# open-rmf/rmf_crowdsim

Hardware: NVIDIA B200
Metric: agent-steps/sec (query+Zanlungo+integrate) (higher is better)
Workload: dtype f64

## Files before the change

### bindings/rust/rmf_crowdsim_gpu-sys/src/lib.rs

```rust
#![allow(non_camel_case_types)]
use std::os::raw::{c_char, c_int};

#[repr(C)]
pub struct rcs_sim {
    _private: [u8; 0],
}

pub const RCS_OK: c_int = 0;
pub const RCS_ERR_OUT_OF_BOUNDS: c_int = 1;
pub const RCS_ERR_SPAWN: c_int = 2;
pub const RCS_ERR_CUDA: c_int = 3;
pub const RCS_ERR_NCCL: c_int = 4;
pub const RCS_ERR_CAPACITY: c_int = 5;
pub const RCS_ERR_ARG: c_int = 6;
pub const RCS_ERR_NO_DEVICE: c_int = 7;
pub const RCS_ERR_HALO: c_int = 8;
pub const RCS_ORDER_STORAGE: u32 = 0;
pub const RCS_ORDER_ID: u32 = 1;
pub const RCS_STEP_DEFAULT: u32 = 0;
pub const RCS_STEP_NO_COMMIT: u32 = 1;

#[repr(C)]
pub struct rcs_sim_desc {
    pub width: f64,
    pub height: f64,
    pub cell_size: f64,
    pub offset_x: f64,
    pub offset_y: f64,
    pub capacity: u64,
    pub device: i32,
    pub flags: u32,
}

#[repr(C)]
#[derive(Default, Debug, Clone, Copy)]
pub struct rcs_stats {
    pub n_agents: u64,
    pub oob_count: u64,
    pub first_oob_id: u64,
    pub nonfinite_count: u64,
    pub finite_tti_count: u64,
    pub neighbour_total: u64,
    pub candidate_total: u64,
    pub spawned: u64,
    pub destroyed: u64,
    pub steps: u64,
}

#[repr(C)]
pub struct rcs_source_sink_desc {
    pub source_x: f64,
    pub source_y: f64,
    pub radius_sink: f64,
    pub monotonic_rate: f64,
    pub hl: u32,
    pub lp: u32,
    pub n_waypoints: u64,
    pub waypoints_xy: *const f64,
    pub loop_forever: i32,
    pub agent_eyesight_range: f64,
}

extern "C" {
    pub fn rcs_abi_version() -> u32;
    pub fn rcs_sim_create(desc: *const rcs_sim_desc, out: *mut *mut rcs_sim) -> c_int;
    pub fn rcs_sim_destroy(sim: *mut rcs_sim);
    pub fn rcs_last_error(sim: *const rcs_sim) -> *const c_char;

    pub fn rcs_lp_none(sim: *mut rcs_sim, out_lp: *mut u32) -> c_int;
    pub fn rcs_lp_zanlungo(sim: *mut rcs_sim, agent_scale: f64, obstacle_scale: f64, reaction_time: f64,
                           force_distance: f64, agent_mass: f64, agent_radius: f64, out_lp: *mut u32) -> c_int;
    pub fn rcs_hl_constant(sim: *mut rcs_sim, vx: f64, vy: f64, out_hl: *mut u32) -> c_int;
    pub fn rcs_hl_parity(sim: *mut rcs_sim, vx: f64, vy: f64, out_hl: *mut u32) -> c_int;
    pub fn rcs_hl_host(sim: *mut rcs_sim, out_hl: *mut u32) -> c_int;
    pub fn rcs_hl_none(sim: *mut rcs_sim, out_hl: *mut u32) -> c_int;
    pub fn rcs_hl_route(sim: *mut rcs_sim, n_points: u64, xy: *const f64, out_hl: *mut u32) -> c_int;
    pub fn rcs_hl_route_set_target(sim: *mut rcs_sim, n: u64, ids: *const u64) -> c_int;
    pub fn rcs_hl_route_table(sim: *mut rcs_sim, n_legs: u64, targets_xy: *const f64, leg_points: *const u64,
                              xy: *const f64, out_hl: *mut u32) -> c_int;
    pub fn rcs_hl_route_table_set_target(sim: *mut rcs_sim, hl: u32, n: u64, ids: *const u64,
                                         targets_xy: *const f64) -> c_int;

    pub fn rcs_add_agents(sim: *mut rcs_sim, n: u64, xy: *const f64, hl: u32, lp: u32, eyesight: f64,
                          out_ids: *mut u64) -> c_int;
    pub fn rcs_remove_agents(sim: *mut rcs_sim, n: u64, ids: *const u64) -> c_int;
    pub fn rcs_set_state(sim: *mut rcs_sim, n: u64, ids: *const u64, x: *const f64, y: *const f64,
                         vx: *const f64, vy: *const f64) -> c_int;
    pub fn rcs_set_preferred_velocity(sim: *mut rcs_sim, n: u64, ids: *const u64, vxy: *const f64) -> c_int;
    pub fn rcs_read_agents(sim: *mut rcs_sim, order: u32, cap: u64, ids: *mut u64, x: *mut f64, y: *mut f64,
                           vx: *mut f64, vy: *mut f64, next_waypoint: *mut u32, out_n: *mut u64) -> c_int;
    pub fn rcs_read_agents_async(sim: *mut rcs_sim, order: u32, cap: u64, ids: *mut u64, x: *mut f64,
                                 y: *mut f64, vx: *mut f64, vy: *mut f64, out_n: *mut u64) -> c_int;
    pub fn rcs_read_wait(sim: *mut rcs_sim) -> c_int;
    pub fn rcs_agent_count(sim: *mut rcs_sim, out_n: *mut u64) -> c_int;

    pub fn rcs_step(sim: *mut rcs_sim, secs: u64, nanos: u32) -> c_int;
    pub fn rcs_step_async(sim: *mut rcs_sim, secs: u64, nanos: u32, flags: u32) -> c_int;
    pub fn rcs_sync(sim: *mut rcs_sim) -> c_int;
    pub fn rcs_step_stats(sim: *mut rcs_sim, out: *mut rcs_stats) -> c_int;
    pub fn rcs_step_in_loop(sim: *mut rcs_sim, secs: u64, nanos: u32, order: *const u64, n_order: u64,
                            max_sweeps: u32, out_sweeps: *mut u32) -> c_int;
    pub fn rcs_poll_events(sim: *mut rcs_sim, spawned_cap: u64, spawned_ids: *mut u64, spawned_xy: *mut f64,
                           n_spawned: *mut u64, destroyed_cap: u64, destroyed_ids: *mut u64,
                           n_destroyed: *mut u64) -> c_int;
    pub fn rcs_add_source_sink(sim: *mut rcs_sim, desc: *const rcs_source_sink_desc, out_id: *mut u64) -> c_int;
    pub fn rcs_remove_source_sink(sim: *mut rcs_sim, id: u64) -> c_int;

    pub fn rcs_cell_of(sim: *mut rcs_sim, n: u64, xy: *const f64, out_idx: *mut i64) -> c_int;
    pub fn rcs_index_add_or_update(sim: *mut rcs_sim, n: u64, ids: *const u64, xy: *const f64) -> c_int;
    pub fn rcs_index_remove(sim: *mut rcs_sim, n: u64, ids: *const u64) -> c_int;
    pub fn rcs_query_radius(sim: *mut rcs_sim, nq: u64, qxy: *const f64, radius: *const f64, offsets: *mut u64,
                            out_ids: *mut u64, ids_cap: u64) -> c_int;
    pub fn rcs_query_knn(sim: *mut rcs_sim, nq: u64, qxy: *const f64, k: u64, out_ids: *mut u64,
                         out_counts: *mut u64) -> c_int;

    pub fn rcs_set_option(sim: *mut rcs_sim, option: u32, value: u64) -> c_int;
    pub fn rcs_graph_stats(sim: *mut rcs_sim, out_graph_launches: *mut u64, out_captures: *mut u64) -> c_int;

    pub fn rcs_nccl_unique_id(out_id: *mut u8) -> c_int;
    pub fn rcs_dist_init(sim: *mut rcs_sim, rank: i32, world: i32, nccl_id: *const u8, halo_capacity: u64) -> c_int;
    pub fn rcs_dist_set_boundaries(sim: *mut rcs_sim, world: i32, bounds: *const u64) -> c_int;
    pub fn rcs_dist_reserve_ids(sim: *mut rcs_sim, next_id: u64) -> c_int;
    pub fn rcs_dist_peer_export(sim: *mut rcs_sim, out_handle: *mut u8) -> c_int;
    pub fn rcs_dist_peer_connect(sim: *mut rcs_sim, left_handle: *const u8, right_handle: *const u8) -> c_int;
    pub fn rcs_dist_peer_disable(sim: *mut rcs_sim) -> c_int;
    pub fn rcs_dist_strip(sim: *mut rcs_sim, rank: i32, world: i32, c0: *mut u64, c1: *mut u64) -> c_int;
    pub fn rcs_dist_add_agents(sim: *mut rcs_sim, n: u64, ids: *const u64, xy: *const f64, vxy: *const f64,
                               hl: u32, lp: u32, eyesight: f64) -> c_int;
}
```

### include/rcs.h

```cpp
#ifndef RCS_H_
#define RCS_H_

#include <stdint.h>

#ifdef __cplusplus
extern "C" {
#endif

#define RCS_ABI_VERSION 1

typedef struct rcs_sim rcs_sim;

enum {
  RCS_OK = 0,
  RCS_ERR_OUT_OF_BOUNDS = 1,
  RCS_ERR_SPAWN = 2,
  RCS_ERR_CUDA = 3,
  RCS_ERR_NCCL = 4,
  RCS_ERR_CAPACITY = 5,
  RCS_ERR_ARG = 6,
  RCS_ERR_NO_DEVICE = 7,
  RCS_ERR_HALO = 8
};

typedef struct rcs_sim_desc {
  double width;
  double height;
  double cell_size;
  double offset_x;
  double offset_y;
  uint64_t capacity;
  int32_t device;
  uint32_t flags;
} rcs_sim_desc;

typedef struct rcs_stats {
  uint64_t n_agents;
  uint64_t oob_count;
  uint64_t first_oob_id;
  uint64_t nonfinite_count;
  uint64_t finite_tti_count;
  uint64_t neighbour_total;
  uint64_t candidate_total;
  uint64_t spawned;
  uint64_t destroyed;
  uint64_t steps;
} rcs_stats;

uint32_t rcs_abi_version(void);

int rcs_sim_create(const rcs_sim_desc* desc, rcs_sim** out);
void rcs_sim_destroy(rcs_sim* sim);
const char* rcs_last_error(const rcs_sim* sim);


int rcs_lp_none(rcs_sim* sim, uint32_t* out_lp);
int rcs_lp_zanlungo(rcs_sim* sim, double agent_scale, double obstacle_scale, double reaction_time,
                    double force_distance, double agent_mass, double agent_radius, uint32_t* out_lp);

int rcs_hl_constant(rcs_sim* sim, double vx, double vy, uint32_t* out_hl);
int rcs_hl_parity(rcs_sim* sim, double vx, double vy, uint32_t* out_hl);
int rcs_hl_host(rcs_sim* sim, uint32_t* out_hl);
int rcs_hl_route(rcs_sim* sim, uint64_t n_points, const double* xy, uint32_t* out_hl);
int rcs_hl_route_set_target(rcs_sim* sim, uint64_t n, const uint64_t* ids);
int rcs_hl_route_table(rcs_sim* sim, uint64_t n_legs, const double* targets_xy, const uint64_t* leg_points,
                       const double* xy, uint32_t* out_hl);
int rcs_hl_route_table_set_target(rcs_sim* sim, uint32_t hl, uint64_t n, const uint64_t* ids,
                                  const double* targets_xy);
int rcs_hl_none(rcs_sim* sim, uint32_t* out_hl);


int rcs_add_agents(rcs_sim* sim, uint64_t n, const double* xy, uint32_t hl, uint32_t lp, double eyesight,
                   uint64_t* out_ids);
int rcs_remove_agents(rcs_sim* sim, uint64_t n, const uint64_t* ids);
int rcs_set_state(rcs_sim* sim, uint64_t n, const uint64_t* ids, const double* x, const double* y,
                  const double* vx, const double* vy);
int rcs_set_preferred_velocity(rcs_sim* sim, uint64_t n, const uint64_t* ids, const double* vxy);

#define RCS_ORDER_STORAGE 0u
#define RCS_ORDER_ID 1u
int rcs_read_agents(rcs_sim* sim, uint32_t order, uint64_t cap, uint64_t* ids, double* x, double* y, double* vx,
                    double* vy, uint32_t* next_waypoint, uint64_t* out_n);
int rcs_agent_count(rcs_sim* sim, uint64_t* out_n);
int rcs_read_agents_async(rcs_sim* sim, uint32_t order, uint64_t cap, uint64_t* ids, double* x, double* y, double* vx,
                          double* vy, uint64_t* out_n);
int rcs_read_wait(rcs_sim* sim);


#define RCS_STEP_DEFAULT 0u
#define RCS_STEP_NO_COMMIT 1u

int rcs_step(rcs_sim* sim, uint64_t secs, uint32_t nanos);
int rcs_step_async(rcs_sim* sim, uint64_t secs, uint32_t nanos, uint32_t flags);
int rcs_sync(rcs_sim* sim);
int rcs_step_stats(rcs_sim* sim, rcs_stats* out);

int rcs_step_in_loop(rcs_sim* sim, uint64_t secs, uint32_t nanos, const uint64_t* order, uint64_t n_order,
                     uint32_t max_sweeps, uint32_t* out_sweeps);

int rcs_poll_events(rcs_sim* sim, uint64_t spawned_cap, uint64_t* spawned_ids, double* spawned_xy,
                    uint64_t* n_spawned, uint64_t destroyed_cap, uint64_t* destroyed_ids, uint64_t* n_destroyed);

typedef struct rcs_source_sink_desc {
  double source_x, source_y;
  double radius_sink;
  double monotonic_rate;
  uint32_t hl, lp;
  uint64_t n_waypoints;
  const double* waypoints_xy;
  int32_t loop_forever;
  double agent_eyesight_range;
} rcs_source_sink_desc;
int rcs_add_source_sink(rcs_sim* sim, const rcs_source_sink_desc* desc, uint64_t* out_id);
int rcs_remove_source_sink(rcs_sim* sim, uint64_t id);


int rcs_cell_of(rcs_sim* sim, uint64_t n, const double* xy, int64_t* out_idx);
int rcs_index_add_or_update(rcs_sim* sim, uint64_t n, const uint64_t* ids, const double* xy);
int rcs_index_remove(rcs_sim* sim, uint64_t n, const uint64_t* ids);
int rcs_query_radius(rcs_sim* sim, uint64_t nq, const double* qxy, const double* radius, uint64_t* offsets,
                     uint64_t* out_ids, uint64_t ids_cap);
int rcs_query_knn(rcs_sim* sim, uint64_t nq, const double* qxy, uint64_t k, uint64_t* out_ids,
                  uint64_t* out_counts);

int rcs_set_trace(rcs_sim* sim, int32_t on);
int rcs_trace_sizes(rcs_sim* sim, uint64_t* n_agents, uint64_t* n_neighbours);
int rcs_read_trace(rcs_sim* sim, uint64_t* ids, double* t_i, double* fx, double* fy, uint64_t* nb_offsets,
                   uint64_t* nb_ids);

#define RCS_OPT_STEP_KERNEL 1u
#define RCS_OPT_GRAPHS 3u
int rcs_set_option(rcs_sim* sim, uint32_t option, uint64_t value);

#define RCS_NUM_EVENTS 64u
int rcs_event_record(rcs_sim* sim, uint32_t slot);
int rcs_event_elapsed_ms(rcs_sim* sim, uint32_t start_slot, uint32_t stop_slot, float* out_ms);
int rcs_host_alloc(uint64_t bytes, void** out);
int rcs_host_free(void* p);
int rcs_flush_l2(rcs_sim* sim, uint64_t bytes);
int rcs_kernel_timing(rcs_sim* sim, int32_t on);
int rcs_kernel_time_ms(rcs_sim* sim, double* out_ms, uint64_t* out_launches);
int rcs_launch_count(rcs_sim* sim, uint64_t* out);
int rcs_graph_stats(rcs_sim* sim, uint64_t* out_graph_launches, uint64_t* out_captures);
int rcs_fp64_peak(int32_t device, double* out_tflops, double* out_dadd_tops);

int rcs_nccl_unique_id(uint8_t out_id[128]);
int rcs_dist_init(rcs_sim* sim, int32_t rank, int32_t world, const uint8_t nccl_id[128], uint64_t halo_capacity);
int rcs_dist_set_boundaries(rcs_sim* sim, int32_t world, const uint64_t* bounds);
int rcs_dist_peer_export(rcs_sim* sim, uint8_t out_handle[64]);
int rcs_dist_peer_connect(rcs_sim* sim, const uint8_t* left_handle, const uint8_t* right_handle);
int rcs_dist_peer_disable(rcs_sim* sim);
int rcs_dist_strip(rcs_sim* sim, int32_t rank, int32_t world, uint64_t* c0, uint64_t* c1);
int rcs_dist_add_agents(rcs_sim* sim, uint64_t n, const uint64_t* ids, const double* xy, const double* vxy,
                        uint32_t hl, uint32_t lp, double eyesight);
int rcs_dist_reserve_ids(rcs_sim* sim, uint64_t next_id);
int rcs_dist_init_local(rcs_sim** sims, int32_t world, uint64_t halo_capacity);
int rcs_dist_step_local(rcs_sim** sims, int32_t world, uint64_t secs, uint32_t nanos, uint32_t flags);

#ifdef __cplusplus
}
#endif
#endif
```

### rmf_crowdsim_b200/_native.py

```python
from __future__ import annotations

import ctypes as C
import os

from . import _build

c_u8p = C.POINTER(C.c_uint8)
c_u32p = C.POINTER(C.c_uint32)
c_u64p = C.POINTER(C.c_uint64)
c_i64p = C.POINTER(C.c_int64)
c_f64p = C.POINTER(C.c_double)
c_f32p = C.POINTER(C.c_float)

RCS_OK = 0
RCS_ERR_OUT_OF_BOUNDS = 1
RCS_ERR_SPAWN = 2
RCS_ERR_CUDA = 3
RCS_ERR_NCCL = 4
RCS_ERR_CAPACITY = 5
RCS_ERR_ARG = 6
RCS_ERR_NO_DEVICE = 7
RCS_ERR_HALO = 8

RCS_ORDER_STORAGE = 0
RCS_ORDER_ID = 1
RCS_STEP_DEFAULT = 0
RCS_STEP_NO_COMMIT = 1
RCS_NUM_EVENTS = 64
RCS_OPT_STEP_KERNEL = 1
RCS_OPT_GRAPHS = 3


class SimDesc(C.Structure):
    _fields_ = [
        ("width", C.c_double),
        ("height", C.c_double),
        ("cell_size", C.c_double),
        ("offset_x", C.c_double),
        ("offset_y", C.c_double),
        ("capacity", C.c_uint64),
        ("device", C.c_int32),
        ("flags", C.c_uint32),
    ]


class Stats(C.Structure):
    _fields_ = [
        ("n_agents", C.c_uint64),
        ("oob_count", C.c_uint64),
        ("first_oob_id", C.c_uint64),
        ("nonfinite_count", C.c_uint64),
        ("finite_tti_count", C.c_uint64),
        ("neighbour_total", C.c_uint64),
        ("candidate_total", C.c_uint64),
        ("spawned", C.c_uint64),
        ("destroyed", C.c_uint64),
        ("steps", C.c_uint64),
    ]


class SourceSinkDesc(C.Structure):
    _fields_ = [
        ("source_x", C.c_double),
        ("source_y", C.c_double),
        ("radius_sink", C.c_double),
        ("monotonic_rate", C.c_double),
        ("hl", C.c_uint32),
        ("lp", C.c_uint32),
        ("n_waypoints", C.c_uint64),
        ("waypoints_xy", c_f64p),
        ("loop_forever", C.c_int32),
        ("agent_eyesight_range", C.c_double),
    ]


SIGNATURES = {
    "rcs_abi_version": (C.c_uint32, []),
    "rcs_sim_create": (C.c_int, [C.POINTER(SimDesc), C.POINTER(C.c_void_p)]),
    "rcs_sim_destroy": (None, [C.c_void_p]),
    "rcs_last_error": (C.c_char_p, [C.c_void_p]),
    "rcs_lp_none": (C.c_int, [C.c_void_p, c_u32p]),
    "rcs_lp_zanlungo": (C.c_int, [C.c_void_p] + [C.c_double] * 6 + [c_u32p]),
    "rcs_hl_constant": (C.c_int, [C.c_void_p, C.c_double, C.c_double, c_u32p]),
    "rcs_hl_parity": (C.c_int, [C.c_void_p, C.c_double, C.c_double, c_u32p]),
    "rcs_hl_host": (C.c_int, [C.c_void_p, c_u32p]),
    "rcs_hl_route": (C.c_int, [C.c_void_p, C.c_uint64, c_f64p, c_u32p]),
    "rcs_hl_route_set_target": (C.c_int, [C.c_void_p, C.c_uint64, c_u64p]),
    "rcs_hl_route_table": (C.c_int, [C.c_void_p, C.c_uint64, c_f64p, c_u64p, c_f64p, c_u32p]),
    "rcs_hl_route_table_set_target": (C.c_int, [C.c_void_p, C.c_uint32, C.c_uint64, c_u64p, c_f64p]),
    "rcs_hl_none": (C.c_int, [C.c_void_p, c_u32p]),
    "rcs_add_agents": (C.c_int, [C.c_void_p, C.c_uint64, c_f64p, C.c_uint32, C.c_uint32, C.c_double, c_u64p]),
    "rcs_remove_agents": (C.c_int, [C.c_void_p, C.c_uint64, c_u64p]),
    "rcs_set_state": (C.c_int, [C.c_void_p, C.c_uint64, c_u64p, c_f64p, c_f64p, c_f64p, c_f64p]),
    "rcs_set_preferred_velocity": (C.c_int, [C.c_void_p, C.c_uint64, c_u64p, c_f64p]),
    "rcs_read_agents": (
        C.c_int,
        [C.c_void_p, C.c_uint32, C.c_uint64, c_u64p, c_f64p, c_f64p, c_f64p, c_f64p, c_u32p, c_u64p],
    ),
    "rcs_agent_count": (C.c_int, [C.c_void_p, c_u64p]),
    "rcs_read_agents_async": (C.c_int, [C.c_void_p, C.c_uint32, C.c_uint64, c_u64p, c_f64p, c_f64p, c_f64p, c_f64p, c_u64p]),
    "rcs_read_wait": (C.c_int, [C.c_void_p]),
    "rcs_step": (C.c_int, [C.c_void_p, C.c_uint64, C.c_uint32]),
    "rcs_step_async": (C.c_int, [C.c_void_p, C.c_uint64, C.c_uint32, C.c_uint32]),
    "rcs_sync": (C.c_int, [C.c_void_p]),
    "rcs_step_stats": (C.c_int, [C.c_void_p, C.POINTER(Stats)]),
    "rcs_step_in_loop": (C.c_int, [C.c_void_p, C.c_uint64, C.c_uint32, c_u64p, C.c_uint64, C.c_uint32, C.POINTER(C.c_uint32)]),
    "rcs_poll_events": (
        C.c_int,
        [C.c_void_p, C.c_uint64, c_u64p, c_f64p, c_u64p, C.c_uint64, c_u64p, c_u64p],
    ),
    "rcs_add_source_sink": (C.c_int, [C.c_void_p, C.POINTER(SourceSinkDesc), c_u64p]),
    "rcs_remove_source_sink": (C.c_int, [C.c_void_p, C.c_uint64]),
    "rcs_cell_of": (C.c_int, [C.c_void_p, C.c_uint64, c_f64p, c_i64p]),
    "rcs_index_add_or_update": (C.c_int, [C.c_void_p, C.c_uint64, c_u64p, c_f64p]),
    "rcs_index_remove": (C.c_int, [C.c_void_p, C.c_uint64, c_u64p]),
    "rcs_query_radius": (C.c_int, [C.c_void_p, C.c_uint64, c_f64p, c_f64p, c_u64p, c_u64p, C.c_uint64]),
    "rcs_query_knn": (C.c_int, [C.c_void_p, C.c_uint64, c_f64p, C.c_uint64, c_u64p, c_u64p]),
    "rcs_set_trace": (C.c_int, [C.c_void_p, C.c_int32]),
    "rcs_trace_sizes": (C.c_int, [C.c_void_p, c_u64p, c_u64p]),
    "rcs_read_trace": (C.c_int, [C.c_void_p, c_u64p, c_f64p, c_f64p, c_f64p, c_u64p, c_u64p]),
    "rcs_set_option": (C.c_int, [C.c_void_p, C.c_uint32, C.c_uint64]),
    "rcs_event_record": (C.c_int, [C.c_void_p, C.c_uint32]),
    "rcs_event_elapsed_ms": (C.c_int, [C.c_void_p, C.c_uint32, C.c_uint32, c_f32p]),
    "rcs_host_alloc": (C.c_int, [C.c_uint64, C.POINTER(C.c_void_p)]),
    "rcs_host_free": (C.c_int, [C.c_void_p]),
    "rcs_flush_l2": (C.c_int, [C.c_void_p, C.c_uint64]),
    "rcs_kernel_timing": (C.c_int, [C.c_void_p, C.c_int32]),
    "rcs_kernel_time_ms": (C.c_int, [C.c_void_p, c_f64p, c_u64p]),
    "rcs_launch_count": (C.c_int, [C.c_void_p, c_u64p]),
    "rcs_graph_stats": (C.c_int, [C.c_void_p, c_u64p, c_u64p]),
    "rcs_fp64_peak": (C.c_int, [C.c_int32, c_f64p, c_f64p]),
    "rcs_nccl_unique_id": (C.c_int, [c_u8p]),
    "rcs_dist_init": (C.c_int, [C.c_void_p, C.c_int32, C.c_int32, c_u8p, C.c_uint64]),
    "rcs_dist_init_local": (C.c_int, [C.POINTER(C.c_void_p), C.c_int32, C.c_uint64]),
    "rcs_dist_step_local": (C.c_int, [C.POINTER(C.c_void_p), C.c_int32, C.c_uint64, C.c_uint32, C.c_uint32]),
    "rcs_dist_strip": (C.c_int, [C.c_void_p, C.c_int32, C.c_int32, c_u64p, c_u64p]),
    "rcs_dist_set_boundaries": (C.c_int, [C.c_void_p, C.c_int32, c_u64p]),
    "rcs_dist_reserve_ids": (C.c_int, [C.c_void_p, C.c_uint64]),
    "rcs_dist_peer_export": (C.c_int, [C.c_void_p, C.POINTER(C.c_uint8)]),
    "rcs_dist_peer_connect": (C.c_int, [C.c_void_p, C.POINTER(C.c_uint8), C.POINTER(C.c_uint8)]),
    "rcs_dist_peer_disable": (C.c_int, [C.c_void_p]),
    "rcs_dist_add_agents": (
        C.c_int,
        [C.c_void_p, C.c_uint64, c_u64p, c_f64p, c_f64p, C.c_uint32, C.c_uint32, C.c_double],
    ),
}

_lib = None


def library_path() -> str:
    return _build.LIB


def load(build_if_missing: bool = True) -> C.CDLL:
    global _lib
    if _lib is not None:
        return _lib
    path = _build.LIB
    if build_if_missing and _build.needs_build():
        try:
            _build.build()
        except Exception as exc:
            if not os.path.exists(path):
                raise RuntimeError(
                    "rmf_crowdsim_b200: the CUDA extension librcs.so is missing and could not be built "
                    f"({exc}).  There is no CPU fallback."
                ) from exc
    if not os.path.exists(path):
        raise RuntimeError(
            "rmf_crowdsim_b200: the CUDA extension librcs.so is missing "
            "(run `python -c 'import __graft_entry__ as g; g.build()'`).  There is no CPU fallback."
        )
    lib = C.CDLL(path)
    for name, (res, args) in SIGNATURES.items():
        fn = getattr(lib, name)
        fn.restype = res
        fn.argtypes = args
    _lib = lib
    return lib


class RcsError(RuntimeError):
# ... 12 lines not shown
```

### rmf_crowdsim_b200/csrc/rcs_host.h

```cpp
#pragma once

#include "../../include/rcs.h"

#include <algorithm>
#include <cmath>
#include <cstdio>
#include <cstdlib>
#include <cstring>
#include <limits>
#include <map>
#include <numeric>
#include <string>
#include <unordered_set>
#include <vector>

#include "rcs_kernels.cuh"
#include "rcs_step_warp.cuh"
#include "rcs_step_tile.cuh"
#include "rcs_inloop.cuh"

namespace rcs_host {

using namespace rcs;

struct LPDesc {
  uint32_t kind;
  double agent_scale, obstacle_scale, reaction_time, force_distance, agent_mass, agent_radius;
};
struct HLDesc {
  uint32_t kind;
  double vx, vy;
  uint32_t route_off, route_n;
  std::map<std::pair<double, double>, uint32_t> legs;
};
inline int64_t leg_of(const HLDesc& h, double x, double y) {
  if (x != x || y != y) return -1;
  const auto it = h.legs.find({x, y});
  return it == h.legs.end() ? -1 : (int64_t)it->second;
}
struct GroupKey {
  uint32_t hl, lp;
  double eyesight;
  int32_t source_sink;
};

struct PendingStep {
  AgentArrays cur, srt;
  bool snapshot_in_srt;
  uint32_t n;
};

struct HaloMem {
  void* base = nullptr;
  uint64_t bytes = 0;
  HaloBuf buf{};
};

struct PeerHalo {
  bool enabled = false;
  void* arena = nullptr;
  uint64_t arena_bytes = 0;
  uint32_t cap = 0;
  void* nb_arena[2] = {nullptr, nullptr};
  HaloBuf remote[2]{};
  uint32_t* remote_hdr[2] = {nullptr, nullptr};
  HaloBuf local[2]{};
  uint32_t* xseq = nullptr;
};

struct Id128 {
  char internal[128];
};
struct NcclApi {
  void* lib = nullptr;
  int (*GetUniqueId)(void*) = nullptr;
  int (*CommInitRank)(void**, int, Id128 , int) = nullptr;
  int (*CommDestroy)(void*) = nullptr;
  int (*Send)(const void*, size_t, int, int, void*, cudaStream_t) = nullptr;
  int (*Recv)(void*, size_t, int, int, void*, cudaStream_t) = nullptr;
  int (*AllReduce)(const void*, void*, size_t, int, int, void*, cudaStream_t) = nullptr;
  int (*GroupStart)() = nullptr;
  int (*GroupEnd)() = nullptr;
  const char* (*GetErrorString)(int) = nullptr;
};

struct StepKey {
  uint64_t epoch = 0, dt_bits = 0;
  const void* cur_pos = nullptr;
  uint32_t flags = 0, n_ub = 0, n = 0;
  uint32_t n_ub_spawn = 0;
  bool cur_has_dead = false;
  bool operator==(const StepKey& o) const {
    return epoch == o.epoch && dt_bits == o.dt_bits && cur_pos == o.cur_pos && flags == o.flags && n_ub == o.n_ub &&
           n == o.n && n_ub_spawn == o.n_ub_spawn && cur_has_dead == o.cur_has_dead;
  }
};
struct StepGraph {
  StepKey key;
  cudaGraphExec_t exec = nullptr;
  uint64_t launches = 0;
};

struct InLoopMem {
  double2 *np_a = nullptr, *np_b = nullptr, *nv = nullptr;
  unsigned long long* rank = nullptr;
  uint32_t *cellid = nullptr, *perm = nullptr, *cell_count = nullptr, *cell_start = nullptr, *cursor = nullptr;
  uint32_t* changed = nullptr;
  uint64_t cap = 0, cells = 0;
};

inline void inloop_free(InLoopMem*& m) {
  if (!m) return;
  cudaFree(m->np_a); cudaFree(m->np_b); cudaFree(m->nv); cudaFree(m->rank); cudaFree(m->cellid); cudaFree(m->perm);
  cudaFree(m->cell_count); cudaFree(m->cell_start); cudaFree(m->cursor); cudaFree(m->changed);
  delete m;
  m = nullptr;
}

}

struct rcs_sim {
  rcs_sim_desc desc{};
  rcs::GridDev grid{};
  int device = 0;
  cudaStream_t stream = nullptr;
  uint64_t cap = 0;
  uint32_t n = 0;
  uint32_t n_ub = 0;
  uint32_t n_tight = 0, n_coarse = 0xffffffffu;
  rcs::AgentArrays cur{}, srt{};
  uint32_t *cellid = nullptr, *perm = nullptr, *cell_count = nullptr, *cell_start = nullptr, *cursor = nullptr;
  uint32_t *tile_sums = nullptr, *scan_total = nullptr, *big_list = nullptr, *slow_list = nullptr, *wide_list = nullptr;
  uint32_t* srt_cell = nullptr;
  rcs::TileRange* tile_ranges = nullptr;
  uint4* slices = nullptr;
  uint32_t* keep = nullptr;
  bool cur_has_dead = false;
  uint64_t tile_sums_cap = 0;
  uint64_t cell_lo = 0, cell_hi = 0;
  uint32_t* cnt = nullptr;
  uint32_t* h_cnt = nullptr;
  bool cnt_dirty = true;
  rcs::GroupDev* d_groups = nullptr;
  uint32_t d_groups_cap = 0;
  std::vector<rcs::GroupDev> groups;
  std::vector<rcs_host::GroupKey> group_keys;
  bool groups_dirty = false;
  std::vector<rcs_host::LPDesc> lps;
  std::vector<rcs_host::HLDesc> hls;
  bool any_zanlungo = false;
  bool any_route = false;
  std::vector<double> routes;
  std::vector<uint32_t> route_end;
  double* d_routes = nullptr;
  uint32_t* d_route_end = nullptr;
  bool routes_dirty = false;
  bool have_host_hl = false;
  rcs::DevStatus* d_status = nullptr;
  rcs::DevStatus* h_status = nullptr;
  uint64_t last_alloc_agent_id = 0;
  unsigned long long* d_next_id = nullptr;
  uint64_t max_id_plus1 = 0;
  bool index_valid = false;
  uint32_t *slot_of_id = nullptr, *id_rank = nullptr, *order_by_id = nullptr, *presence = nullptr;
  uint64_t slot_table_cap = 0;
  bool slot_valid = false;
  bool trace = false;
  double *tr_ti = nullptr, *tr_fx = nullptr, *tr_fy = nullptr;
  uint32_t *tr_nbc = nullptr, *tr_nbo = nullptr, *tr_own = nullptr;
  uint64_t *tr_nbids = nullptr, *tr_id = nullptr;
  uint64_t tr_nbids_cap = 0, tr_nb_total = 0;
  uint32_t tr_n = 0;
  bool tr_valid = false;
  std::vector<rcs::SourceSinkDev> sources;
  std::vector<double> ss_wp;
  std::vector<uint32_t> ss_rwp;
  rcs::SourceSinkDev* d_sources = nullptr;
  double* d_ss_wp = nullptr;
  uint32_t* d_ss_rwp = nullptr;
  uint32_t* d_blocked = nullptr;
  uint32_t *d_ss_bits_local = nullptr, *d_ss_bits_parts = nullptr, *d_ss_bits = nullptr;
  uint32_t ss_words = 0;
  cudaEvent_t ev_flags = nullptr;
  uint32_t *d_sg_start = nullptr, *d_sg_items = nullptr;
  rcs::SourceGridDev sgrid{};
  bool sources_dirty = false;
  uint32_t n_sources_alive = 0;
  bool ever_had_sources = false;
  unsigned long long *ev_spawn_id = nullptr, *ev_destroyed = nullptr;
  double* ev_spawn_xy = nullptr;
  uint32_t ev_cap = 0;
  rcs::StripDev strip{};
  int rank = 0, world = 1;
  uint32_t halo_width = 0;
  std::vector<uint64_t> strip_bounds;
  rcs_host::HaloMem send_l, send_r, recv_l, recv_r;
  rcs_host::PeerHalo peer;
  void* nccl_comm = nullptr;
  std::vector<rcs_sim*> local_group;
  cudaEvent_t ev_packed = nullptr, ev_copied = nullptr;
  void* stage = nullptr;
  uint64_t stage_bytes = 0;
  cudaStream_t copy_stream = nullptr;
  cudaEvent_t ev_gathered = nullptr, ev_read_done = nullptr;
  void* stage2 = nullptr;
  uint64_t stage2_bytes = 0;
  bool read_inflight = false;
  cudaEvent_t ev_half_done[2] = {nullptr, nullptr};
  bool half_used[2] = {false, false};
  uint64_t read_seq = 0;
  cudaStream_t up_stream = nullptr;
  cudaEvent_t ev_uploaded = nullptr, ev_pv_scattered = nullptr;
  void* pv_stage = nullptr;
  uint64_t pv_stage_bytes = 0;
  bool pv_inflight = false;
  rcs_host::InLoopMem* inloop = nullptr;
  void* flush_buf = nullptr;
  uint64_t flush_bytes = 0;
  unsigned int* d_bad = nullptr;
  unsigned long long* d_bad2 = nullptr;
  std::vector<rcs_host::PendingStep> pending;
  uint64_t steps_enqueued = 0;
  unsigned long long* d_steps_done = nullptr;
  uint64_t steps_done_at_sync = 0;
  std::string err;
  uint64_t launches = 0;
  rcs_stats stats{};
  cudaEvent_t events[RCS_NUM_EVENTS]{};
  uint32_t opt_step_kernel = 0;
  bool tile_attr_set = false;
  uint32_t opt_graphs = 1;
  uint64_t graph_epoch = 0;
  std::vector<rcs_host::StepGraph> step_graphs;
  rcs_host::StepKey recent_keys[2];
  uint64_t graph_launches = 0, graph_captures = 0;
  bool ktiming = false;
  std::vector<std::pair<cudaEvent_t, cudaEvent_t>> kevents;
  std::vector<cudaEvent_t> kevent_pool;
  double ktime_ms = 0.0;
  uint64_t ktime_n = 0;
};

namespace rcs_host {

extern thread_local std::string g_create_error;

#define CU_TRY(sim, call)                                                                         \
  do {                                                                                            \
    cudaError_t e__ = (call);                                                                     \
    if (e__ != cudaSuccess) {                                                                     \
      (sim)->err = std::string("CUDA error: ") + cudaGetErrorString(e__) + " at " #call;          \
      return RCS_ERR_CUDA;                                                                        \
    }                                                                                             \
  } while (0)

inline uint32_t blocks_for(uint64_t n, uint32_t threads) {
  return (uint32_t)std::max<uint64_t>((n + threads - 1) / threads, 1);
}

template <class T>
inline cudaError_t dalloc(T** p, uint64_t count) {
  return cudaMalloc(reinterpret_cast<void**>(p), std::max<uint64_t>(count, 1) * sizeof(T));
}

inline bool churn(const rcs_sim* s) { return s->ever_had_sources || s->strip.enabled; }

}
```

### rmf_crowdsim_b200/csrc/rcs_kernels.cuh

```cuda
#pragma once

#include "rcs_math.cuh"

namespace rcs {

struct DevStatus {
  unsigned int oob_count;
  unsigned int nonfinite_count;
  unsigned int big_cells;
  unsigned int failed;
  unsigned int local_failed;
  unsigned int halo_err;
  unsigned int capacity_err;
  unsigned int spawned;
  unsigned int destroyed;
  unsigned int slow_count;
  unsigned int wide_count;
  unsigned int sort_ticket;
  unsigned long long first_oob_id;
  unsigned long long finite_tti;
  unsigned long long neighbour_total;
  unsigned long long candidate_total;
};

// ... 120 lines not shown
    GridDev g, uint32_t n_ub, const uint32_t* __restrict__ last, const double2* __restrict__ pos,
    const uint32_t* __restrict__ keep, uint32_t* __restrict__ cellid, uint32_t* __restrict__ cell_count,
    uint64_t cell_lo, uint64_t cell_hi, PackArgs pk, DevStatus* status) {
  if (status->failed) return;
  const uint32_t i = blockIdx.x * blockDim.x + threadIdx.x;
  bool live = i < n_ub && i < *last;
  if (!PACK && !live) return;
  if (live && keep && !keep[i]) {
    cellid[i] = CELL_DEAD;
    live = false;
    if (!PACK) return;
  }
  uint64_t idx = 0;
  if (live) live = bin_one(g, i, pos[i], cellid, cell_count, cell_lo, cell_hi, status, idx);
  if (PACK) halo_pack_block<BIN_THREADS>(pk, live, i, (uint32_t)idx, status);
}

__device__ __forceinline__ uint32_t warp_inclusive_scan(uint32_t v) {
  const unsigned lane = threadIdx.x & 31u;
#pragma unroll
  for (int d = 1; d < 32; d <<= 1) {
    uint32_t t = __shfl_up_sync(0xffffffffu, v, d);
    if (lane >= (unsigned)d) v += t;
  }
  return v;
}

__device__ __forceinline__ uint32_t block_exclusive_scan(uint32_t v, uint32_t& total) {
  constexpr int NW = SCAN_THREADS / 32;
  __shared__ uint32_t warp_off[NW];
  __shared__ uint32_t s_total;
  const unsigned lane = threadIdx.x & 31u, warp = threadIdx.x >> 5;
  uint32_t inc = warp_inclusive_scan(v);
  if (lane == 31) warp_off[warp] = inc;
  __syncthreads();
  if (warp == 0) {
    uint32_t w = lane < NW ? warp_off[lane] : 0u;
    uint32_t winc = warp_inclusive_scan(w);
    if (lane < NW) warp_off[lane] = winc - w;
    if (lane == NW - 1) s_total = winc;
  }
  __syncthreads();
  total = s_total;
  uint32_t r = warp_off[warp] + inc - v;
  __syncthreads();
  return r;
}

__global__ void scan_reduce_kernel(const uint32_t* __restrict__ in, uint64_t len, uint32_t* __restrict__ tile_sums) {
  uint64_t base = (uint64_t)blockIdx.x * SCAN_TILE + (uint64_t)threadIdx.x * SCAN_ITEMS;
  uint32_t s = 0;
  if (base + SCAN_ITEMS <= len) {
    const uint4* p = reinterpret_cast<const uint4*>(in + base);
#pragma unroll
    for (int k = 0; k < SCAN_ITEMS / 4; ++k) {
      uint4 v = p[k];
      s += v.x + v.y + v.z + v.w;
    }
  } else {
    for (int k = 0; k < SCAN_ITEMS; ++k)
      if (base + k < len) s += in[base + k];
  }
  uint32_t total;
  (void)block_exclusive_scan(s, total);
  if (threadIdx.x == 0) tile_sums[blockIdx.x] = total;
}

__global__ void scan_tile_sums_kernel(uint32_t* __restrict__ tile_sums, uint32_t n_tiles, uint32_t* total_out) {
  uint32_t carry = 0;
  for (uint32_t base = 0; base < n_tiles; base += SCAN_THREADS) {
    uint32_t i = base + threadIdx.x;
    uint32_t v = i < n_tiles ? tile_sums[i] : 0u;
    uint32_t total;
    uint32_t ex = block_exclusive_scan(v, total);
    if (i < n_tiles) tile_sums[i] = carry + ex;
    carry += total;
    __syncthreads();
  }
  if (threadIdx.x == 0) *total_out = carry;
}

template <bool RAW_SUMS>
__global__ void scan_apply_kernel(const uint32_t* __restrict__ in, uint64_t len,
                                  const uint32_t* __restrict__ tile_sums, uint32_t* __restrict__ cell_start,
                                  uint32_t* __restrict__ cursor) {
  uint64_t base = (uint64_t)blockIdx.x * SCAN_TILE + (uint64_t)threadIdx.x * SCAN_ITEMS;
  uint32_t v[SCAN_ITEMS];
  uint32_t s = 0;
  if (base + SCAN_ITEMS <= len) {
    const uint4* p = reinterpret_cast<const uint4*>(in + base);
#pragma unroll
    for (int k = 0; k < SCAN_ITEMS / 4; ++k) {
      uint4 q = p[k];
      v[4 * k + 0] = q.x;
      v[4 * k + 1] = q.y;
      v[4 * k + 2] = q.z;
      v[4 * k + 3] = q.w;
    }
  } else {
#pragma unroll
    for (int k = 0; k < SCAN_ITEMS; ++k) v[k] = (base + k < len) ? in[base + k] : 0u;
  }
#pragma unroll
  for (int k = 0; k < SCAN_ITEMS; ++k) s += v[k];
  uint32_t total, before;
  if (RAW_SUMS) {
    uint32_t part = 0;
    for (uint32_t t = threadIdx.x; t < blockIdx.x; t += SCAN_THREADS) part += tile_sums[t];
    (void)block_exclusive_scan(part, before);
  } else {
    before = tile_sums[blockIdx.x];
  }
  uint32_t run = before + block_exclusive_scan(s, total);
  if (base + SCAN_ITEMS <= len) {
    uint32_t o[SCAN_ITEMS];
#pragma unroll
    for (int k = 0; k < SCAN_ITEMS; ++k) {
      o[k] = run;
      run += v[k];
    }
    uint4* ps = reinterpret_cast<uint4*>(cell_start + base);
    uint4* pc = reinterpret_cast<uint4*>(cursor + base);
#pragma unroll
    for (int k = 0; k < SCAN_ITEMS / 4; ++k) {
      uint4 q = make_uint4(o[4 * k], o[4 * k + 1], o[4 * k + 2], o[4 * k + 3]);
      ps[k] = q;
      if (cursor) pc[k] = q;
    }
    if (base + SCAN_ITEMS == len) cell_start[len] = run;
  } else {
    for (int k = 0; k < SCAN_ITEMS; ++k) {
      if (base + k < len) {
        cell_start[base + k] = run;
        if (cursor) cursor[base + k] = run;
        run += v[k];
        if (base + k + 1 == len) cell_start[len] = run;
      }
    }
  }
}

__global__ void scatter_perm_kernel(uint32_t n_ub, const uint32_t* __restrict__ n_ptr,
                                    const uint32_t* __restrict__ cellid, uint32_t* __restrict__ cursor,
                                    uint32_t* __restrict__ perm, const DevStatus* status) {
  if (status->failed) return;
  uint32_t i = blockIdx.x * blockDim.x + threadIdx.x;
  if (i >= n_ub || i >= *n_ptr) return;
  uint32_t c = cellid[i];
  if (c == CELL_DEAD) return;
  uint32_t pos = atomicAdd(&cursor[c], 1u);
  perm[pos] = i;
}

__global__ void sort_cells_by_id_kernel(uint64_t cell_lo, uint64_t cell_hi, const uint32_t* __restrict__ cell_start,
                                        const uint64_t* __restrict__ id, uint32_t* __restrict__ perm,
                                        uint32_t* __restrict__ big_list, uint32_t big_cap, DevStatus* status) {
  if (status->failed) return;
  uint64_t c = cell_lo + (uint64_t)blockIdx.x * blockDim.x + threadIdx.x;
  if (c >= cell_hi) return;
  uint32_t s = cell_start[c], e = cell_start[c + 1];
  uint32_t m = e - s;
  if (m < 2) return;
  if (m > SORT_LOCAL_MAX) {
    uint32_t k = atomicAdd(&status->big_cells, 1u);
    if (k < big_cap) big_list[k] = (uint32_t)c;
    return;
  }
  uint32_t p[SORT_LOCAL_MAX];
  uint64_t key[SORT_LOCAL_MAX];
  bool sorted = true;
  for (uint32_t k = 0; k < m; ++k) {
    p[k] = perm[s + k];
    key[k] = id[p[k]];
    if (k && key[k] < key[k - 1]) sorted = false;
  }
  if (sorted) return;
  for (uint32_t k = 1; k < m; ++k) {
    uint32_t pk = p[k];
    uint64_t kk = key[k];
    int j = (int)k - 1;
    while (j >= 0 && key[j] > kk) {
      key[j + 1] = key[j];
      p[j + 1] = p[j];
      --j;
    }
    key[j + 1] = kk;
    p[j + 1] = pk;
  }
  for (uint32_t k = 0; k < m; ++k) perm[s + k] = p[k];
}

constexpr uint32_t BIG_SMEM_KEYS = 4096;

__device__ __forceinline__ void sort_one_big_cell(uint32_t s, uint32_t e, const uint64_t* __restrict__ id,
                                                  uint32_t* __restrict__ perm, uint32_t* __restrict__ scratch,
                                                  uint32_t* __restrict__ ranks, unsigned long long* skeys) {
  const uint32_t m = e - s;
  for (uint32_t t0 = 0; t0 < m; t0 += BIG_SMEM_KEYS) {
    const uint32_t tl = min(BIG_SMEM_KEYS, m - t0);
    __syncthreads();
    for (uint32_t j = threadIdx.x; j < tl; j += blockDim.x) skeys[j] = id[perm[s + t0 + j]];
    __syncthreads();
    for (uint32_t k = threadIdx.x; k < m; k += blockDim.x) {
      const uint64_t kk = id[perm[s + k]];
      uint32_t rank = t0 ? ranks[s + k] : 0u;
      for (uint32_t j = 0; j < tl; ++j) rank += (skeys[j] < kk) ? 1u : 0u;
      ranks[s + k] = rank;
    }
  }
  for (uint32_t k = threadIdx.x; k < m; k += blockDim.x) scratch[s + ranks[s + k]] = perm[s + k];
  __syncthreads();
  for (uint32_t k = s + threadIdx.x; k < e; k += blockDim.x) perm[k] = scratch[k];
  __syncthreads();
}

constexpr uint32_t HUGE_ELEMS = 64;

__device__ __forceinline__ void rank_huge_cell(uint32_t s, uint32_t e, const uint64_t* __restrict__ id,
                                               const uint32_t* __restrict__ perm, uint32_t* __restrict__ scratch,
                                               unsigned long long* skeys, uint32_t (*partial)[HUGE_ELEMS]) {
  const uint32_t m = e - s;
  const uint32_t warp = threadIdx.x >> 5, lane = threadIdx.x & 31u, nwarps = blockDim.x >> 5;
  for (uint32_t k0 = blockIdx.x * HUGE_ELEMS; k0 < m; k0 += gridDim.x * HUGE_ELEMS) {
    const uint32_t kA = k0 + lane, kB = k0 + lane + 32u;
    const uint64_t keyA = kA < m ? id[perm[s + kA]] : 0ull, keyB = kB < m ? id[perm[s + kB]] : 0ull;
    uint32_t rA = 0, rB = 0;
    for (uint32_t t0 = 0; t0 < m; t0 += BIG_SMEM_KEYS) {
      const uint32_t tl = min(BIG_SMEM_KEYS, m - t0);
      __syncthreads();
      for (uint32_t j = threadIdx.x; j < tl; j += blockDim.x) skeys[j] = id[perm[s + t0 + j]];
      __syncthreads();
      for (uint32_t j = warp; j < tl; j += nwarps) {
        const uint64_t key = skeys[j];
        rA += (key < keyA) ? 1u : 0u;
        rB += (key < keyB) ? 1u : 0u;
      }
    }
    partial[warp][lane] = rA;
    partial[warp][lane + 32u] = rB;
    __syncthreads();
    if (threadIdx.x < HUGE_ELEMS && k0 + threadIdx.x < m) {
      uint32_t rank = 0;
      for (uint32_t w = 0; w < nwarps; ++w) rank += partial[w][threadIdx.x];
      scratch[s + rank] = perm[s + k0 + threadIdx.x];
    }
    __syncthreads();
  }
}

__global__ void __launch_bounds__(1024) sort_big_cells_kernel(uint64_t cell_lo, uint64_t cell_hi,
                                                              const uint32_t* __restrict__ cell_start,
                                                              const uint64_t* __restrict__ id,
                                                              uint32_t* __restrict__ perm,
                                                              uint32_t* __restrict__ scratch,
                                                              uint32_t* __restrict__ ranks,
                                                              const uint32_t* __restrict__ big_list, uint32_t big_cap,
                                                              DevStatus* status) {
  __shared__ unsigned long long skeys[BIG_SMEM_KEYS];
  __shared__ uint32_t partial[32][HUGE_ELEMS];
  __shared__ bool last_block;
  if (status->failed) return;
  const uint32_t nbig = status->big_cells;
  if (nbig <= big_cap) {
    for (uint32_t b = blockIdx.x; b < nbig; b += gridDim.x) {
      const uint32_t c = big_list[b];
      const uint32_t cs = cell_start[c], ce = cell_start[c + 1];
      if (ce - cs <= BIG_SMEM_KEYS) sort_one_big_cell(cs, ce, id, perm, scratch, ranks, skeys);
    }
    uint32_t n_huge = 0;
    for (uint32_t b = 0; b < nbig; ++b) {
      const uint32_t c = big_list[b];
      const uint32_t cs = cell_start[c], ce = cell_start[c + 1];
      if (ce - cs > BIG_SMEM_KEYS) {
        rank_huge_cell(cs, ce, id, perm, scratch, skeys, partial);
        n_huge += 1;
      }
    }
    if (n_huge) {
      __threadfence();
      __syncthreads();
      if (threadIdx.x == 0) last_block = atomicAdd(&status->sort_ticket, 1u) == gridDim.x - 1;
      __syncthreads();
      if (last_block) {
        __threadfence();
        for (uint32_t b = 0; b < nbig; ++b) {
          const uint32_t c = big_list[b];
          const uint32_t cs = cell_start[c], ce = cell_start[c + 1];
          if (ce - cs > BIG_SMEM_KEYS)
            for (uint32_t k = cs + threadIdx.x; k < ce; k += blockDim.x) perm[k] = __ldcg(scratch + k);
        }
        if (threadIdx.x == 0) status->sort_ticket = 0u;
      }
    }
  } else {
    for (uint64_t c = cell_lo + blockIdx.x; c < cell_hi; c += gridDim.x) {
      const uint32_t cs = cell_start[c], ce = cell_start[c + 1];
      if (ce - cs > SORT_LOCAL_MAX) sort_one_big_cell(cs, ce, id, perm, scratch, ranks, skeys);
    }
  }
}

__device__ __forceinline__ uint4 query_slices(const GridDev& g, const uint32_t* __restrict__ cell_start,
                                              const GroupDev& gr, double px, double py) {
  uint4 sl = make_uint4(0u, 0u, 0u, 0u);
  if (gr.lp_kind == LP_ZANLUNGO) {
    int64_t left, right, bottom, top;
    get_bounds(g, gr.eyesight, px, py, left, right, bottom, top);
    if (left < 0) left = 0;
    if (right > g.x_max) right = g.x_max;
    if (right - left <= 2) {
      uint32_t st[3] = {0, 0, 0}, ln[3] = {0, 0, 0};
#pragma unroll
      for (int c = 0; c < 3; ++c) {
        uint64_t c_lo, c_hi;
        if (left + c <= right && column_cell_range(g, left + c, bottom, top, c_lo, c_hi)) {
          st[c] = cell_start[c_lo];
          const uint32_t l = cell_start[c_hi + 1] - st[c];
          ln[c] = l > 255u ? 255u : l;
        }
      }
      sl = make_uint4(st[0], st[1], st[2], ln[0] | (ln[1] << 8) | (ln[2] << 16) | (1u << 24));
    }
  }
  return sl;
}

struct TileRange {
  uint32_t lo[3];
  uint32_t len[3];
};
__device__ __forceinline__ bool st_takes(const GroupDev& g, uint64_t id, uint4 sl);
__device__ __forceinline__ void st_block_ranges(bool takes, uint4 sl, uint32_t (*red)[6], TileRange* out);
#ifndef RCS_TILE_WARPS
#define RCS_TILE_WARPS 4
#endif
constexpr int ST_WARPS = RCS_TILE_WARPS;
constexpr int GATHER_THREADS = 32 * ST_WARPS;

__global__ void __launch_bounds__(GATHER_THREADS) gather_sorted_kernel(
    uint32_t n, const uint32_t* __restrict__ perm, AgentArrays cur, AgentArrays srt, const uint32_t* __restrict__ cellid,
    uint32_t* __restrict__ srt_cell, const uint32_t* __restrict__ n_sorted, GridDev g,
    const uint32_t* __restrict__ cell_start, const GroupDev* __restrict__ groups, uint4* __restrict__ slices,
    TileRange* __restrict__ tile_ranges, const DevStatus* status) {
  __shared__ uint32_t red[GATHER_THREADS / 32][6];
  if (status->failed) return;
  const uint32_t k = blockIdx.x * blockDim.x + threadIdx.x;
  bool takes = false;
  uint4 sl = make_uint4(0u, 0u, 0u, 0u);
  if (k < n && k < *n_sorted) {
    const uint32_t i = perm[k];
    const double2 p = cur.pos[i];
    const uint32_t grp = cur.grp[i];
    const uint64_t id = cur.id[i];
    if (srt_cell) srt_cell[k] = cellid[i];
    srt.pos[k] = p;
    srt.vel[k] = cur.vel[i];
    srt.id[k] = id;
    srt.grp[k] = grp;
    srt.wp[k] = cur.wp[i];
    if (cur.pv) srt.pv[k] = cur.pv[i];
    if (slices) {
      sl = query_slices(g, cell_start, groups[grp], p.x, p.y);
      slices[k] = sl;
      takes = st_takes(groups[grp], id, sl);
    }
  }
  if (tile_ranges) st_block_ranges(takes, sl, red, tile_ranges + blockIdx.x);
}

struct StepArgs {
  GridDev grid;
  uint32_t n;
  const uint32_t* n_sorted;
  AgentArrays in;
  const uint32_t* cell_start;
  const GroupDev* groups;
  double dt;
  double2 *opos, *ovel;
  uint64_t* oid;
  uint32_t *ogrp, *owp;
  double2* opv;
  double *t_i, *fx, *fy;
  uint32_t* nb_count;
  uint64_t* tr_id;
  uint32_t* tr_own;
  DevStatus* status;
  uint32_t collect_stats;
  uint32_t no_commit;
  const unsigned long long* steps_done;
  uint32_t* keep;
  const uint32_t* cell;
  StripDev strip;
  const SourceSinkDev* ss;
  const double* ss_wp;
  const uint32_t* ss_rwp;
  uint32_t* cnt;
  unsigned long long* ev_destroyed;
  uint32_t ev_cap;
  uint32_t* slow_list;
  uint32_t* wide_list;
  const uint4* slices;
  const TileRange* tile_ranges;
  const double* routes;
  const uint32_t* route_end;
  double route_thr2;
};

constexpr uint32_t WP_MASK = 0xffffu;
constexpr int WP_ROUTE_SHIFT = 16;

enum : uint32_t { ROLE_PASSIVE = 0, ROLE_OWN = 1, ROLE_RING = 2, ROLE_MASK = 3,
                  ROLE_NEAR_L = 1u << 8, ROLE_NEAR_R = 1u << 9, ROLE_HAS_NEAR = 1u << 10 };

__device__ __forceinline__ uint32_t agent_role_of_cell(const StepArgs& a, uint32_t cell) {
  if (!a.strip.enabled) return ROLE_OWN;
  const uint32_t cx = cell / (uint32_t)a.grid.nx;
  if (cx >= a.strip.c0 && cx < a.strip.c1) return ROLE_OWN;
  if (cx + a.strip.h >= a.strip.c0 && cx < a.strip.c1 + a.strip.h) return ROLE_RING;
  return ROLE_PASSIVE;
}
__device__ __forceinline__ uint32_t agent_role_and_bits(const StepArgs& a, uint32_t cell) {
  const uint32_t cx = cell / (uint32_t)a.grid.nx;
  uint32_t r = ROLE_PASSIVE;
  if (cx >= a.strip.c0 && cx < a.strip.c1) r = ROLE_OWN;
  else if (cx + a.strip.h >= a.strip.c0 && cx < a.strip.c1 + a.strip.h) r = ROLE_RING;
  if (cx < a.strip.c0 + a.strip.h) r |= ROLE_NEAR_L;
  if (cx + a.strip.h >= a.strip.c1) r |= ROLE_NEAR_R;
  return r | ROLE_HAS_NEAR;
}
__device__ __forceinline__ uint32_t agent_role(const StepArgs& a, uint32_t i) {
  return a.strip.enabled ? agent_role_of_cell(a, a.cell[i]) : (uint32_t)ROLE_OWN;
}

__device__ __forceinline__ void drop_entry(const StepArgs& a, uint32_t i) {
  if (a.keep) a.keep[i] = 0u;
}

struct Self {
  double px, py, vx, vy, pfx, pfy;
  uint64_t id;
  uint32_t rwp;
};

template <class F>
__device__ __forceinline__ uint32_t for_each_neighbour(const GridDev& g, const uint32_t* __restrict__ cell_start,
                                                       const double2* __restrict__ pos,
                                                       const uint64_t* __restrict__ ids, double px, double py,
                                                       uint64_t self_id, double radius, double thr2, F&& f) {
  int64_t left, right, bottom, top;
  get_bounds(g, radius, px, py, left, right, bottom, top);
  if (left < 0) left = 0;
  if (right > g.x_max) right = g.x_max;
  uint32_t cand = 0;
  for (int64_t cx = left; cx <= right; ++cx) {
    uint64_t c_lo, c_hi;
    if (!column_cell_range(g, cx, bottom, top, c_lo, c_hi)) continue;
    uint32_t s = cell_start[c_lo], e = cell_start[c_hi + 1];
    cand += e - s;
    for (uint32_t j = s; j < e; ++j) {
      const double2 q = pos[j];
      double dx = q.x - px;
      double dy = q.y - py;
      double d2 = dx * dx + dy * dy;
      if (d2 < thr2) {
        if (ids[j] != self_id) f(j, dx, dy, d2);
      }
    }
  }
  return cand;
}

__device__ __noinline__ void zanlungo_sequential(const StepArgs& a, uint32_t i, const Self& me, const GroupDev& g,
                                                 double& t_i, double& fx, double& fy, uint32_t& nbc,
                                                 uint32_t& cand) {
  const double2* __restrict__ pos = a.in.pos;
  const double2* __restrict__ vel = a.in.vel;
  const uint64_t* __restrict__ ids = a.in.id;
  const double rr = g.rr;
  t_i = RCS_INF;
  fx = 0.0;
  fy = 0.0;
  cand = for_each_neighbour(a.grid, a.cell_start, pos, ids, me.px, me.py, me.id, g.eyesight, g.thr2,
                            [&](uint32_t j, double dx, double dy, double d2) {
                              nbc++;
                              const double2 nv = vel[j];
                              double col_time = time_to_collision(nv.x - me.vx, nv.y - me.vy, dx, dy, d2, rr);
                              if (col_time < t_i) t_i = col_time;
                            });
  if (t_i != RCS_INF) {
    const OwnerPre pre = owner_precompute(me.px, me.py, me.vx, me.vy, me.pfx, me.pfy, t_i, g);
    const double ti = t_i;
    for_each_neighbour(a.grid, a.cell_start, pos, ids, me.px, me.py, me.id, g.eyesight, g.thr2,
// ... 873 lines not shown
```

Before: 5.119 billion.

## Add incremental grid rebuild that rebins only agents whose cell changed

Adds an incremental spatial-grid rebuild path. When agents are already stored in sorted cell order, each agent's new cell is compared with its previous cell, and counts are adjusted atomically. Cells that no agent entered or left get an identity permutation, so only changed cells are re-sorted by id. It also sets a min-blocks launch bound on the gather kernel. The aim is to avoid a full counting sort every step, at the cost of atomics, extra state (moved/slot), and a more complex graph key. The host-side wiring is not shown.

```diff
diff --git a/bindings/rust/rmf_crowdsim_gpu-sys/src/lib.rs b/bindings/rust/rmf_crowdsim_gpu-sys/src/lib.rs
--- a/bindings/rust/rmf_crowdsim_gpu-sys/src/lib.rs
+++ b/bindings/rust/rmf_crowdsim_gpu-sys/src/lib.rs
@@ -19,6 +19,9 @@
 pub const RCS_ORDER_ID: u32 = 1;
 pub const RCS_STEP_DEFAULT: u32 = 0;
 pub const RCS_STEP_NO_COMMIT: u32 = 1;
+pub const RCS_OPT_STEP_KERNEL: u32 = 1;
+pub const RCS_OPT_GRAPHS: u32 = 3;
+pub const RCS_OPT_REBUILD: u32 = 5;
 
 #[repr(C)]
 pub struct rcs_sim_desc {
diff --git a/include/rcs.h b/include/rcs.h
--- a/include/rcs.h
+++ b/include/rcs.h
@@ -130,6 +130,7 @@
 
 #define RCS_OPT_STEP_KERNEL 1u
 #define RCS_OPT_GRAPHS 3u
+#define RCS_OPT_REBUILD 5u
 int rcs_set_option(rcs_sim* sim, uint32_t option, uint64_t value);
 
 #define RCS_NUM_EVENTS 64u
diff --git a/rmf_crowdsim_b200/_native.py b/rmf_crowdsim_b200/_native.py
--- a/rmf_crowdsim_b200/_native.py
+++ b/rmf_crowdsim_b200/_native.py
@@ -29,6 +29,7 @@
 RCS_NUM_EVENTS = 64
 RCS_OPT_STEP_KERNEL = 1
 RCS_OPT_GRAPHS = 3
+RCS_OPT_REBUILD = 5
 
 
 class SimDesc(C.Structure):
diff --git a/rmf_crowdsim_b200/csrc/rcs_host.h b/rmf_crowdsim_b200/csrc/rcs_host.h
--- a/rmf_crowdsim_b200/csrc/rcs_host.h
+++ b/rmf_crowdsim_b200/csrc/rcs_host.h
@@ -90,9 +90,10 @@
   uint32_t flags = 0, n_ub = 0, n = 0;
   uint32_t n_ub_spawn = 0;
   bool cur_has_dead = false;
+  bool cur_sorted = false;
   bool operator==(const StepKey& o) const {
     return epoch == o.epoch && dt_bits == o.dt_bits && cur_pos == o.cur_pos && flags == o.flags && n_ub == o.n_ub &&
-           n == o.n && n_ub_spawn == o.n_ub_spawn && cur_has_dead == o.cur_has_dead;
+           n == o.n && n_ub_spawn == o.n_ub_spawn && cur_has_dead == o.cur_has_dead && cur_sorted == o.cur_sorted;
   }
 };
 struct StepGraph {
@@ -132,6 +133,9 @@
   uint32_t *cellid = nullptr, *perm = nullptr, *cell_count = nullptr, *cell_start = nullptr, *cursor = nullptr;
   uint32_t *tile_sums = nullptr, *scan_total = nullptr, *big_list = nullptr, *slow_list = nullptr, *wide_list = nullptr;
   uint32_t* srt_cell = nullptr;
+  bool cur_sorted = false;
+  uint32_t* moved = nullptr;
+  uint32_t* slot = nullptr;
   rcs::TileRange* tile_ranges = nullptr;
   uint4* slices = nullptr;
   uint32_t* keep = nullptr;
@@ -228,6 +232,7 @@
   rcs_stats stats{};
   cudaEvent_t events[RCS_NUM_EVENTS]{};
   uint32_t opt_step_kernel = 0;
+  uint32_t opt_rebuild = 0;
   bool tile_attr_set = false;
   uint32_t opt_graphs = 1;
   uint64_t graph_epoch = 0;
@@ -265,4 +270,6 @@
 
 inline bool churn(const rcs_sim* s) { return s->ever_had_sources || s->strip.enabled; }
 
-}
+inline bool incremental_rebuild(const rcs_sim* s) { return s->opt_rebuild == 0 && !churn(s); }
+
+}
diff --git a/rmf_crowdsim_b200/csrc/rcs_kernels.cuh b/rmf_crowdsim_b200/csrc/rcs_kernels.cuh
--- a/rmf_crowdsim_b200/csrc/rcs_kernels.cuh
+++ b/rmf_crowdsim_b200/csrc/rcs_kernels.cuh
@@ -296,13 +296,9 @@
   perm[pos] = i;
 }
 
-__global__ void sort_cells_by_id_kernel(uint64_t cell_lo, uint64_t cell_hi, const uint32_t* __restrict__ cell_start,
-                                        const uint64_t* __restrict__ id, uint32_t* __restrict__ perm,
-                                        uint32_t* __restrict__ big_list, uint32_t big_cap, DevStatus* status) {
-  if (status->failed) return;
-  uint64_t c = cell_lo + (uint64_t)blockIdx.x * blockDim.x + threadIdx.x;
-  if (c >= cell_hi) return;
-  uint32_t s = cell_start[c], e = cell_start[c + 1];
+__device__ __forceinline__ void sort_cell_by_id(uint64_t c, uint32_t s, uint32_t e, const uint64_t* __restrict__ id,
+                                                uint32_t* __restrict__ perm, uint32_t* __restrict__ big_list,
+                                                uint32_t big_cap, DevStatus* status) {
   uint32_t m = e - s;
   if (m < 2) return;
   if (m > SORT_LOCAL_MAX) {
@@ -332,6 +328,15 @@
     p[j + 1] = pk;
   }
   for (uint32_t k = 0; k < m; ++k) perm[s + k] = p[k];
+}
+
+__global__ void sort_cells_by_id_kernel(uint64_t cell_lo, uint64_t cell_hi, const uint32_t* __restrict__ cell_start,
+                                        const uint64_t* __restrict__ id, uint32_t* __restrict__ perm,
+                                        uint32_t* __restrict__ big_list, uint32_t big_cap, DevStatus* status) {
+  if (status->failed) return;
+  uint64_t c = cell_lo + (uint64_t)blockIdx.x * blockDim.x + threadIdx.x;
+  if (c >= cell_hi) return;
+  sort_cell_by_id(c, cell_start[c], cell_start[c + 1], id, perm, big_list, big_cap, status);
 }
 
 constexpr uint32_t BIG_SMEM_KEYS = 4096;
@@ -442,6 +447,98 @@
       if (ce - cs > SORT_LOCAL_MAX) sort_one_big_cell(cs, ce, id, perm, scratch, ranks, skeys);
     }
   }
+}
+
+constexpr uint32_t CELL_LEFT = 0x80000000u;
+constexpr int REBIN_THREADS = 256;
+
+__device__ __forceinline__ uint32_t insert_cell(const GridDev& g, double2 x) {
+  uint64_t idx;
+  return location_to_index(g, x.x, x.y, idx) ? (uint32_t)idx : CELL_DEAD;
+}
+
+__device__ __forceinline__ void rebin_row(const GridDev& g, uint32_t i, double2 x, uint32_t p,
+                                          uint32_t* __restrict__ cell_count, uint32_t* __restrict__ moved,
+                                          uint32_t* __restrict__ slot, DevStatus* status) {
+  const uint32_t c = insert_cell(g, x);
+  if (c == CELL_DEAD) atomicAdd(&status->oob_count, 1u);
+  if (c == p) return;
+  if (p != CELL_DEAD) {
+    atomicSub(&cell_count[p], 1u);
+    atomicOr(&moved[p], CELL_LEFT);
+  }
+  if (c != CELL_DEAD) {
+    atomicAdd(&cell_count[c], 1u);
+    slot[i] = atomicAdd(&moved[c], 1u) & ~CELL_LEFT;
+  }
+}
+
+__global__ void __launch_bounds__(REBIN_THREADS) rebin_kernel(
+    GridDev g, uint32_t n_ub, const uint32_t* __restrict__ last, const double2* __restrict__ pos,
+    const uint32_t* __restrict__ cell_start, uint32_t* __restrict__ prev_start, uint32_t* __restrict__ cell_count,
+    uint32_t* __restrict__ moved, uint32_t* __restrict__ slot, uint64_t cell_lo, uint64_t cell_hi,
+    DevStatus* status) {
+  if (status->failed) return;
+  const uint32_t t = blockIdx.x * blockDim.x + threadIdx.x;
+  const uint64_t len = cell_hi - cell_lo, c = cell_lo + t;
+  if (t <= len) {
+    const uint32_t r = cell_start[c];
+    prev_start[c] = r;
+    const uint32_t e = t < len ? cell_start[c + 1] : r;
+    for (uint32_t k = r; k < e; k += 4) {
+      double2 x[4];
+#pragma unroll
+      for (int j = 0; j < 4; ++j)
+        if (k + j < e) x[j] = pos[k + j];
+#pragma unroll
+      for (int j = 0; j < 4; ++j)
+        if (k + j < e) rebin_row(g, k + j, x[j], (uint32_t)c, cell_count, moved, slot, status);
+    }
+  }
+  const uint32_t n = min(n_ub, *last);
+  for (uint32_t i = cell_start[cell_hi] + t; i < n; i += gridDim.x * blockDim.x)
+    rebin_row(g, i, pos[i], CELL_DEAD, cell_count, moved, slot, status);
+}
+
+__global__ void place_movers_kernel(GridDev g, uint32_t n_ub, const uint32_t* __restrict__ last, uint64_t cell_lo,
+                                    uint64_t cell_hi, const uint32_t* __restrict__ cell_start,
+                                    const uint32_t* __restrict__ prev_start, const uint32_t* __restrict__ moved,
+                                    const double2* __restrict__ pos, const uint32_t* __restrict__ slot,
+                                    uint32_t* __restrict__ perm, const DevStatus* status) {
+  if (status->failed) return;
+  const uint32_t t = blockIdx.x * blockDim.x + threadIdx.x;
+  const uint64_t c = cell_lo + t;
+  if (c < cell_hi && moved[c]) {
+    uint32_t k = cell_start[c];
+    for (uint32_t r = prev_start[c]; r < prev_start[c + 1]; ++r) {
+      const uint32_t nc = insert_cell(g, pos[r]);
+      if (nc == (uint32_t)c)
+        perm[k++] = r;
+      else if (nc != CELL_DEAD)
+        perm[cell_start[nc + 1] - 1 - slot[r]] = r;
+    }
+  }
+  const uint32_t n = min(n_ub, *last);
+  for (uint32_t i = prev_start[cell_hi] + t; i < n; i += gridDim.x * blockDim.x) {
+    const uint32_t nc = insert_cell(g, pos[i]);
+    if (nc != CELL_DEAD) perm[cell_start[nc + 1] - 1 - slot[i]] = i;
+  }
+}
+
+__global__ void place_cells_kernel(uint64_t cell_lo, uint64_t cell_hi, const uint32_t* __restrict__ cell_start,
+                                   const uint32_t* __restrict__ prev_start, uint32_t* __restrict__ moved,
+                                   const uint64_t* __restrict__ id, uint32_t* __restrict__ perm,
+                                   uint32_t* __restrict__ big_list, uint32_t big_cap, DevStatus* status) {
+  if (status->failed) return;
+  const uint64_t c = cell_lo + (uint64_t)blockIdx.x * blockDim.x + threadIdx.x;
+  if (c >= cell_hi) return;
+  const uint32_t s = cell_start[c], e = cell_start[c + 1], ps = prev_start[c];
+  if (!moved[c]) {
+    for (uint32_t k = 0; k < e - s; ++k) perm[s + k] = ps + k;
+    return;
+  }
+  moved[c] = 0u;
+  sort_cell_by_id(c, s, e, id, perm, big_list, big_cap, status);
 }
 
 __device__ __forceinline__ uint4 query_slices(const GridDev& g, const uint32_t* __restrict__ cell_start,
@@ -481,7 +578,7 @@
 constexpr int ST_WARPS = RCS_TILE_WARPS;
 constexpr int GATHER_THREADS = 32 * ST_WARPS;
 
-__global__ void __launch_bounds__(GATHER_THREADS) gather_sorted_kernel(
+__global__ void __launch_bounds__(GATHER_THREADS, 16) gather_sorted_kernel(
     uint32_t n, const uint32_t* __restrict__ perm, AgentArrays cur, AgentArrays srt, const uint32_t* __restrict__ cellid,
     uint32_t* __restrict__ srt_cell, const uint32_t* __restrict__ n_sorted, GridDev g,
     const uint32_t* __restrict__ cell_start, const GroupDev* __restrict__ groups, uint4* __restrict__ slices,
```

Measured after the change: 5.357 billion (median of 6 runs). +4.7%, better.
